# python-microscopy/ch-shrinkwrap

Hardware: NVIDIA B200
Metric: localisation_iterations_per_s (higher is better)
Workload: dtype f32 (fp64 nearest-face compare and Gram sums, int64 fixed-point adjoint)

## Files before the change

ch_shrinkwrap_b200/csrc/common.cuh:

```cuda
#pragma once
#include <cuda_runtime.h>
#include <cfloat>
#include <stdint.h>
#include <string>
#include <unordered_map>
#include <vector>
#include "../../include/nanowrap.h"

#define NW_MAX_LEVELS 12
#define NW_MAX_ITERS 4096
#define NW_S2_PTS 4
#define NW_N_STAGES 11

#ifdef NW_BOUNDS_CHECK
#include <cassert>
#define NW_ASSERT(c) assert(c)
#else
#define NW_ASSERT(c) ((void)0)
#endif

struct Box {
    float4 a;
    float4 b;
    float4 c;
// ... 108 lines not shown
    int64_t P_global = 0;
    float *px = nullptr, *py = nullptr, *pz = nullptr;
    double *px64 = nullptr, *py64 = nullptr, *pz64 = nullptr;
    float *sx = nullptr, *sy = nullptr, *sz = nullptr;
    float *wx = nullptr, *wy = nullptr, *wz = nullptr;
    float sinv_scalar = 1.f;
    int reg_mode = 0;
    int weights_mode = 0;
    float wmean = 1.f;
    int has_mask = 0;
    uint8_t *pmask = nullptr;
    int *perm = nullptr;
    int *slot = nullptr;
    float *w0 = nullptr, *w1 = nullptr, *w2 = nullptr;
    float *rx = nullptr, *ry = nullptr, *rz = nullptr;
    float bbox_pts[6] = {0, 0, 0, 0, 0, 0};
    double wn_max = 1.0;
    bool weights_valid = false;

    int M = 0, F = 0;
    float4 *posq = nullptr, *nrmq = nullptr;
    int *faces = nullptr;
    int *nbrT = nullptr;
    int *valence = nullptr;
    uint8_t *valid = nullptr;
    int *stage_nbr = nullptr, *stage_hev = nullptr;
    int *tb_small = nullptr, *tb_i0 = nullptr, *tb_i1 = nullptr;
    unsigned *tb_u0 = nullptr, *tb_u1 = nullptr, *tb_u2 = nullptr;
    int4 *sfaces = nullptr;
    float4 *cent = nullptr;
    Box *boxes = nullptr;
    int *parent_g = nullptr; int2 *kids = nullptr;
    int *leaf_of_slot = nullptr;
    float *node_f = nullptr;
    TreeLevels tl;
    bool seeds_cold = true;
    float *fx = nullptr, *fy = nullptr, *fz = nullptr;
    bool feet_valid = false;
    unsigned *fkeys = nullptr;
    int *fkey_tab = nullptr;
    float key_lo[3] = {0, 0, 0}, key_inv = 0.f;
    unsigned *fcells = nullptr;
    bool points_mode = false;
    double *cent64 = nullptr;
    Box *tboxes = nullptr;
    char *surf_q = nullptr;
    unsigned *surf_bits = nullptr;
    double *surf_dist = nullptr, *surf_closest = nullptr, *surf_part = nullptr;
    int *surf_face = nullptr;
    int64_t topo_gen = 0;
    int64_t sgn_gen = -1;
    int sgn_defects[5] = {0, 0, 0, 0, 0};
    int *sgn_twin = nullptr;
    int *sgn_voff = nullptr, *sgn_vface = nullptr;
    unsigned long long *sgn_k0 = nullptr, *sgn_k1 = nullptr;
    int *sgn_i0 = nullptr, *sgn_i1 = nullptr;
    int *sgn_cnt = nullptr;
    double *sgn_nv = nullptr;
    double *sgn_vpart = nullptr;
    unsigned *sgn_bbox = nullptr;
    uint8_t *sx_flag = nullptr;
    int *sx_last = nullptr;
    unsigned long long *sx_keys = nullptr, *sx_sorted = nullptr;
    unsigned long long *sx_cnt = nullptr;
    int2 *sx_pairs = nullptr;
    unsigned long long *acc = nullptr;
    float4 *Sq = nullptr;
// ... 145 lines not shown
```

ch_shrinkwrap_b200/csrc/tree.cu:

```cuda
#include <cub/cub.cuh>
#include <cfloat>
#include "common.cuh"
#include <thread>
#include <vector>

namespace {

__device__ __forceinline__ float3 centroid_f32(const float4 a, const float4 b, const float4 c) {
    float3 r;
    r.x = __fdiv_rn(__fadd_rn(__fadd_rn(a.x, b.x), c.x), 3.0f);
    r.y = __fdiv_rn(__fadd_rn(__fadd_rn(a.y, b.y), c.y), 3.0f);
    r.z = __fdiv_rn(__fadd_rn(__fadd_rn(a.z, b.z), c.z), 3.0f);
    return r;
}

__global__ void k_pack_vec3(const float *__restrict__ src, int M, float4 *__restrict__ dst) {
    int i = blockIdx.x * blockDim.x + threadIdx.x;
    if (i < M) dst[i] = make_float4(src[3 * i], src[3 * i + 1], src[3 * i + 2], 0.f);
}

__global__ void k_unpack_vec3(const float4 *__restrict__ src, int M, float *__restrict__ dst) {
    int i = blockIdx.x * blockDim.x + threadIdx.x;
    if (i < M) { float4 v = src[i]; dst[3 * i] = v.x; dst[3 * i + 1] = v.y; dst[3 * i + 2] = v.z; }
}
// ... 39 lines not shown
    return points ? make_float3(a.x, a.y, a.z) : centroid_f32(a, b, c);
}

__global__ void k_face_bbox(const int *__restrict__ faces, const float4 *__restrict__ pos, int F, int *__restrict__ out6, bool points) {
    float lo[3] = {FLT_MAX, FLT_MAX, FLT_MAX}, hi[3] = {-FLT_MAX, -FLT_MAX, -FLT_MAX};
    for (int f = blockIdx.x * blockDim.x + threadIdx.x; f < F; f += gridDim.x * blockDim.x) {
        float3 c = centroid_of(points, pos[faces[3 * f]], pos[faces[3 * f + 1]], pos[faces[3 * f + 2]]);
        float v[3] = {c.x, c.y, c.z};
        for (int a = 0; a < 3; ++a) if (v[a] == v[a]) { lo[a] = fminf(lo[a], v[a]); hi[a] = fmaxf(hi[a], v[a]); }
    }
    for (int a = 0; a < 3; ++a)
        for (int o = 16; o; o >>= 1) {
            lo[a] = fminf(lo[a], __shfl_xor_sync(0xffffffffu, lo[a], o));
            hi[a] = fmaxf(hi[a], __shfl_xor_sync(0xffffffffu, hi[a], o));
        }
    if ((threadIdx.x & 31) == 0)
        for (int a = 0; a < 3; ++a) {
            int l = __float_as_int(lo[a]); l = l >= 0 ? l : l ^ 0x7fffffff;
            int u = __float_as_int(hi[a]); u = u >= 0 ? u : u ^ 0x7fffffff;
            atomicMin(out6 + a, l);
            atomicMax(out6 + 3 + a, u);
        }
}

__device__ __forceinline__ unsigned spread10(unsigned v) {
    v &= 0x3ffu;
    v = (v | v << 16) & 0x30000ffu;
    v = (v | v << 8) & 0x300f00fu;
    v = (v | v << 4) & 0x30c30c3u;
    v = (v | v << 2) & 0x9249249u;
    return v;
}

__global__ void k_face_keys(const int *__restrict__ faces, const float4 *__restrict__ pos, int F, float3 lo, float inv,
                            unsigned *__restrict__ keys, int *__restrict__ idx, unsigned *__restrict__ cells, bool points) {
    int f = blockIdx.x * blockDim.x + threadIdx.x;
    if (f >= F) return;
    float3 c = centroid_of(points, pos[faces[3 * f]], pos[faces[3 * f + 1]], pos[faces[3 * f + 2]]);
    unsigned qx = (unsigned)fminf(fmaxf((c.x - lo.x) * inv, 0.f), 1023.f);
    unsigned qy = (unsigned)fminf(fmaxf((c.y - lo.y) * inv, 0.f), 1023.f);
    unsigned qz = (unsigned)fminf(fmaxf((c.z - lo.z) * inv, 0.f), 1023.f);
    cells[f] = qx | (qy << 10) | (qz << 20);
    hilbert_axes_to_transpose(qx, qy, qz, 10);
    keys[f] = (spread10(qx) << 2) | (spread10(qy) << 1) | spread10(qz);
    idx[f] = f;
}

__global__ void k_sorted_faces(const int *__restrict__ faces, const int *__restrict__ order, int F, int4 *__restrict__ sfaces,
                               const unsigned *__restrict__ cells, unsigned *__restrict__ fcells) {
    int i = blockIdx.x * blockDim.x + threadIdx.x;
    if (i >= F) return;
    int f = order[i];
    sfaces[i] = make_int4(faces[3 * f], faces[3 * f + 1], faces[3 * f + 2], f);
    fcells[i] = cells[f];
}

__device__ __forceinline__ void project3(const float3 n, const float4 c, float &pn, float &p1, float &p2) {
    const float3 t1 = nw_tangent_of(n.x, n.y, n.z);
    const float3 t2 = make_float3(n.y * t1.z - n.z * t1.y, n.z * t1.x - n.x * t1.z, n.x * t1.y - n.y * t1.x);
    pn = fmaf(n.x, c.x, fmaf(n.y, c.y, n.z * c.z));
    p1 = fmaf(t1.x, c.x, fmaf(t1.y, c.y, t1.z * c.z));
    p2 = fmaf(t2.x, c.x, fmaf(t2.y, c.y, t2.z * c.z));
}


__global__ void k_level_histogram(const unsigned *__restrict__ keys, int F, int *__restrict__ hist) {
    const int i = blockIdx.x * blockDim.x + threadIdx.x;
    int lvl = 0;
    if (i < F && i > 0) {
        const unsigned x = keys[i] ^ keys[i - 1];
        if (x) lvl = (29 - (31 - __clz(x))) / 3 + 1;
    }
    for (int k = 1; k <= 10; ++k) {
        const unsigned m = __ballot_sync(0xffffffffu, lvl == k);
        if (m && (threadIdx.x & 31) == 0) atomicAdd(&hist[k], __popc(m));
    }
}

__global__ void k_level_flags(const unsigned *__restrict__ keys, int F, int shift, int *__restrict__ flag) {
    const int i = blockIdx.x * blockDim.x + threadIdx.x;
    if (i >= F) return;
    flag[i] = (i == 0) ? 1 : (shift >= 32 ? 0 : ((keys[i] >> shift) != (keys[i - 1] >> shift)));
}

__device__ __forceinline__ bool ends_node(const unsigned *__restrict__ keys, int F, int lvl, int i) {
    return i == F - 1 || ((keys[i] ^ keys[i + 1]) >> (30 - 3 * lvl)) != 0;
}

__global__ void k_level_tables(const unsigned *__restrict__ keys, int F, int lvl, int off_up, const int *__restrict__ id_up,
                               const int *__restrict__ start_up, int off, const int *__restrict__ id, int *__restrict__ start,
                               int *__restrict__ parent_g, int2 *__restrict__ kids, Box *__restrict__ boxes,
                               int *__restrict__ leaf_of_slot) {
    const int i = blockIdx.x * blockDim.x + threadIdx.x;
    if (i >= F) return;
    if (!id) leaf_of_slot[i] = id_up[i] - 1;
    else if (i == 0 || id[i - 1] != id[i]) start[id[i] - 1] = i;
    if (lvl < 0 || !ends_node(keys, F, lvl, i)) return;
    const int p = off_up + id_up[i] - 1, s0 = start_up[id_up[i] - 1];
    const int c0 = id ? off + id[s0] - 1 : s0, c1 = id ? off + id[i] - 1 : i;
    const unsigned last = (lvl == 0 || ends_node(keys, F, lvl - 1, i)) ? 0x80000000u : 0u;
    kids[p] = make_int2(c0, c1 - c0 + 1);
    boxes[p].d.z = __int_as_float((int)((unsigned)c0 | last));
    if (id) for (int c = c0; c <= c1; ++c) parent_g[c] = (int)((unsigned)p | last);
    if (lvl == 0) parent_g[0] = (int)0x80000000u;
}

__global__ void k_refit_centroids(const int4 *__restrict__ sfaces, const float4 *__restrict__ pos, int F, float4 *__restrict__ cent,
                                  const unsigned *__restrict__ fcells, float3 lo, float inv, SolverState *st, bool points) {
    const int i = blockIdx.x * blockDim.x + threadIdx.x;
    float esc = 0.f;
    if (i < F) {
        const int4 sf = sfaces[i];
        const float3 cc = centroid_of(points, pos[sf.x], pos[sf.y], pos[sf.z]);
        cent[i] = make_float4(cc.x, cc.y, cc.z, __int_as_float(sf.w));
        const unsigned cell = fcells[i];
        const float gx = (cc.x - lo.x) * inv, gy = (cc.y - lo.y) * inv, gz = (cc.z - lo.z) * inv;
        const float cx = (float)(cell & 1023u), cy = (float)((cell >> 10) & 1023u), cz = (float)(cell >> 20);
        esc = fmaxf(fmaxf(fmaxf(cx - gx, cx == 1023.f ? 0.f : gx - (cx + 1.f)), fmaxf(cy - gy, cy == 1023.f ? 0.f : gy - (cy + 1.f))),
                    fmaxf(fmaxf(cz - gz, cz == 1023.f ? 0.f : gz - (cz + 1.f)), 0.f));
        if (!(esc >= 0.f)) esc = __int_as_float(0x7f800000);
    }
    const unsigned m = __reduce_max_sync(0xffffffffu, __float_as_uint(esc));
    if ((threadIdx.x & 31) == 0 && m) atomicMax((unsigned *)&st->cell_escape, m);
}

__global__ void __launch_bounds__(256) k_leaf_normals(const int4 *__restrict__ sfaces, const float4 *__restrict__ pos, int F,
                                                      const int *__restrict__ leaf_of_slot, int leaf0, float *__restrict__ nsum) {
    const int i = blockIdx.x * blockDim.x + threadIdx.x;
    if (i >= F) return;
    const int4 sf = sfaces[i];
    const float4 a = pos[sf.x], b = pos[sf.y], d = pos[sf.z];
    const float ux = b.x - a.x, uy = b.y - a.y, uz = b.z - a.z, vx = d.x - a.x, vy = d.y - a.y, vz = d.z - a.z;
    float3 fn = make_float3(uy * vz - uz * vy, uz * vx - ux * vz, ux * vy - uy * vx);
    if (!(fabsf(fn.x) <= FLT_MAX && fabsf(fn.y) <= FLT_MAX && fabsf(fn.z) <= FLT_MAX)) return;
    float *dst = nsum + 3 * (size_t)(leaf0 + leaf_of_slot[i]);
    atomicAdd(dst, fn.x); atomicAdd(dst + 1, fn.y); atomicAdd(dst + 2, fn.z);
}
__global__ void __launch_bounds__(256) k_up_normals(float *__restrict__ nsum, const int2 *__restrict__ kids, int first, int count) {
    const int j = blockIdx.x * blockDim.x + threadIdx.x;
    if (j >= count) return;
    const int2 k = kids[first + j];
    float sx = 0.f, sy = 0.f, sz = 0.f;
    for (int c = k.x; c < k.x + k.y; ++c) {
        const float *s = nsum + 3 * (size_t)c;
        sx += s[0]; sy += s[1]; sz += s[2];
    }
    float *d = nsum + 3 * (size_t)(first + j);
    d[0] = sx; d[1] = sy; d[2] = sz;
}

__global__ void k_key_table(const unsigned *__restrict__ fkeys, int F, int *__restrict__ tab) {
    const int b = blockIdx.x * blockDim.x + threadIdx.x;
    if (b > 32768) return;
    const unsigned long long key = (unsigned long long)b << 15;
    int lo = 0, hi = F;
    while (lo < hi) {
        const int mid = (lo + hi) >> 1;
        if ((unsigned long long)fkeys[mid] < key) lo = mid + 1; else hi = mid;
    }
    tab[b] = lo;
}

__global__ void k_node_frames(Box *__restrict__ boxes, const float *__restrict__ nsum, int first, int count) {
    const int j = blockIdx.x * blockDim.x + threadIdx.x;
    if (j >= count) return;
    const float *s = nsum + 3 * (size_t)(first + j);
    float3 n = make_float3(s[0], s[1], s[2]);
    const float nn = sqrtf(n.x * n.x + n.y * n.y + n.z * n.z);
    n = (nn > 1e-20f && nn <= FLT_MAX) ? make_float3(n.x / nn, n.y / nn, n.z / nn) : make_float3(0.f, 0.f, 1.f);
    Box *b = &boxes[first + j];
    const float3 t1 = nw_tangent_of(n.x, n.y, n.z);
    b->a = make_float4(n.x, t1.x, n.y, t1.y);
    b->b = make_float4(n.z, t1.z, NW_EMPTY_LO, NW_EMPTY_LO);
    b->c = make_float4(n.y * t1.z - n.z * t1.y, n.z * t1.x - n.x * t1.z, n.x * t1.y - n.y * t1.x, NW_EMPTY_HI);
    b->d.x = NW_EMPTY_HI; b->d.y = NW_EMPTY_HI; b->d.w = NW_EMPTY_LO;
}

__global__ void k_reset_extents(Box *__restrict__ boxes, int first, int count) {
    const int j = blockIdx.x * blockDim.x + threadIdx.x;
    if (j >= count) return;
    Box *b = &boxes[first + j];
    b->b.z = NW_EMPTY_LO; b->b.w = NW_EMPTY_LO; b->d.w = NW_EMPTY_LO; b->d.x = NW_EMPTY_HI; b->d.y = NW_EMPTY_HI; b->c.w = NW_EMPTY_HI;
}

__global__ void __launch_bounds__(256) k_extents(const float4 *__restrict__ cent, int F, const int *__restrict__ leaf_of_slot,
                                                 int leaf0, int leaf_level, const int *__restrict__ parent_g, Box *__restrict__ boxes) {
    const int i = blockIdx.x * blockDim.x + threadIdx.x;
    const bool live = i < F;
    const float4 c = live ? cent[i] : make_float4(0.f, 0.f, 0.f, 0.f);
    const bool finite = live && (c.x == c.x) && (c.y == c.y) && (c.z == c.z);
    int node = live ? leaf0 + leaf_of_slot[i] : 0;
    for (int l = leaf_level; l >= 1; --l) {
        nw_merge_extents(boxes, node, live, finite, [&](const Box *b, float (&lo)[3], float (&hi)[3]) {
            const float4 ba = b->a;
            project3(make_float3(ba.x, ba.z, b->b.x), c, lo[0], lo[1], lo[2]);
            hi[0] = lo[0]; hi[1] = lo[1]; hi[2] = lo[2];
        });
        if (live) node = parent_g[node] & 0x7fffffff;
    }
}
__global__ void k_box_decode(Box *__restrict__ boxes, int first, int count, const SolverState *__restrict__ st) {
    int i = blockIdx.x * blockDim.x + threadIdx.x;
    if (i >= count) return;
    nw_decode_box(&boxes[first + i], st->coord_l1 * 1.9073486328125e-6f);
}

#define NW_NMOM 3

inline float ordered_to_float(int v) {
    v = v >= 0 ? v : v ^ 0x7fffffff;
    float f;
    memcpy(&f, &v, 4);
    return f;
}

}

static int set_topology_impl(nw_ctx *h, const float *pos, const float *nrm, const int32_t *faces, const int32_t *nbr,
                             const int32_t *he_vertex, int n_he, const uint8_t *valid, int M, int F, int he_stride = 4);

extern "C" int nw_set_topology(nw_ctx *h, const float *pos, const float *nrm, const int32_t *faces,
                               const int32_t *nbr, const uint8_t *valid, int M, int F) {
    return set_topology_impl(h, pos, nrm, faces, nbr, nullptr, 0, valid, M, F);
}

extern "C" int nw_set_topology_halfedge(nw_ctx *h, const float *pos, const float *nrm, const int32_t *faces,
                                        const int32_t *nbr_halfedge, const int32_t *he_vertex, int n_halfedges,
                                        const uint8_t *valid, int M, int F) {
    if (h && !(he_vertex && n_halfedges > 0)) { h->err = "nw_set_topology_halfedge: missing half-edge table"; return NW_ERR_ARG; }
    return set_topology_impl(h, pos, nrm, faces, nbr_halfedge, he_vertex, n_halfedges, valid, M, F);
}

extern "C" int nw_set_topology_records(nw_ctx *h, const void *vertex_records, const int32_t *faces, const int32_t *he_vertex,
                                       int he_stride_bytes, int n_halfedges, int M, int F) {
    if (h && !(vertex_records && he_vertex && n_halfedges > 0)) { h->err = "nw_set_topology_records: NULL array"; return NW_ERR_ARG; }
    if (h && !(he_stride_bytes >= 4 && he_stride_bytes % 4 == 0)) { h->err = "nw_set_topology_records: he_stride_bytes must be a multiple of 4"; return NW_ERR_ARG; }
    return set_topology_impl(h, (const float *)vertex_records, nullptr, faces, nullptr, he_vertex, n_halfedges, nullptr, M, F, he_stride_bytes);
}

static int seg_begin(nw_ctx *h) {
// ... 72 lines not shown
        NW_CHECK(nw_alloc(h, &h->stage_nbr, (size_t)NW_NEIGHBORSIZE * M));
        NW_CHECK(nw_upload_replicated(h, h->scratchM, pos, sizeof(float) * 3 * (size_t)M));
        NW_CHECK(seg_begin(h));
        k_pack_vec3<<<nw_grid(M, B), B, 0, s>>>(h->scratchM, M, h->posq);
        h->launches += 1;
        NW_CHECK(seg_end(h));
        NW_CUDA(cudaStreamSynchronize(s));
        NW_CHECK(nw_upload_replicated(h, h->scratchM, nrm, sizeof(float) * 3 * (size_t)M));
        NW_CHECK(seg_begin(h));
        k_pack_vec3<<<nw_grid(M, B), B, 0, s>>>(h->scratchM, M, h->nrmq);
        h->launches += 1;
        NW_CHECK(seg_end(h));
        NW_CHECK(nw_upload_replicated(h, h->stage_nbr, nbr, sizeof(int) * NW_NEIGHBORSIZE * (size_t)M));
        NW_CHECK(seg_begin(h));
        k_transpose_nbr<<<nw_grid(M, B), B, 0, s>>>(h->stage_nbr, he_vertex ? h->stage_hev : nullptr, n_he, M, h->nbrT, h->valence);
        h->launches += 1;
        NW_CHECK(seg_end(h));
        if (valid) NW_CHECK(nw_upload_replicated(h, h->valid, valid, (size_t)M));
        else NW_CUDA(cudaMemsetAsync(h->valid, 1, M, s));
    }
    }
    NW_CUDA(cudaStreamSynchronize(s));
    NW_CHECK(seg_begin(h));
    NW_CUDA(cudaMemsetAsync(h->acc, 0, sizeof(unsigned long long) * 4 * M, s));
    NW_CUDA(cudaMemsetAsync(h->Sq, 0, sizeof(float4) * 3 * M, s));
    if (h->slot && h->P) NW_CUDA(cudaMemsetAsync(h->slot, 0xff, sizeof(int) * h->P, s));
    h->seeds_cold = true;
    h->order_stale = true;
    NW_CHECK(nw_tree_build(h));
    NW_CHECK(seg_end(h));
    return nw_comm_agree(h);
}

static int scan_inclusive(nw_ctx *h, const int *in, int *out, int n) {
    size_t tmp = 0;
    cub::DeviceScan::InclusiveSum(nullptr, tmp, in, out, n, h->stream);
    if (tmp > h->cub_tmp_bytes) { NW_CHECK(nw_alloc(h, (char **)&h->cub_tmp, tmp)); h->cub_tmp_bytes = tmp; }
    NW_CUDA(cub::DeviceScan::InclusiveSum(h->cub_tmp, tmp, in, out, n, h->stream));
    h->launches += 2;
    return NW_OK;
}

static int extents_pass(nw_ctx *h) {
    cudaStream_t s = h->stream;
    const int B = 256;
    const TreeLevels &tl = h->tl;
    const int first = tl.off[1], count = tl.off[tl.n_levels - 1] + tl.count[tl.n_levels - 1] - first;
    k_reset_extents<<<nw_grid(count, B), B, 0, s>>>(h->boxes, first, count);
    NW_LAUNCH_CHECK();
    k_extents<<<nw_grid(h->F, B), B, 0, s>>>(h->cent, h->F, h->leaf_of_slot, tl.off[tl.n_levels - 1], tl.n_levels - 1, h->parent_g,
                                             h->boxes);
    NW_LAUNCH_CHECK();
    k_box_decode<<<nw_grid(count, B), B, 0, s>>>(h->boxes, first, count, h->st);
    NW_LAUNCH_CHECK();
    return NW_OK;
}

static void launch_refit_centroids(nw_ctx *h) {
    cudaMemsetAsync(&h->st->cell_escape, 0, sizeof(float), h->stream);
    k_refit_centroids<<<nw_grid(h->F, 256), 256, 0, h->stream>>>(h->sfaces, h->posq, h->F, h->cent, h->fcells,
                                                                 make_float3(h->key_lo[0], h->key_lo[1], h->key_lo[2]), h->key_inv, h->st,
                                                                 h->points_mode);
}

int nw_tree_refit(nw_ctx *h) {
    launch_refit_centroids(h);
    NW_LAUNCH_CHECK();
    return extents_pass(h);
}

int nw_tree_build(nw_ctx *h) {
    cudaStream_t s = h->stream;
    const int B = 256, F = h->F;
    int *&d_bbox = h->tb_small, *&idx = h->tb_i0, *&order = h->tb_i1;
    unsigned *&keys = h->tb_u0, *&keys2 = h->tb_u1;
    NW_CHECK(nw_alloc(h, &d_bbox, 16));
    int init[6] = {0x7fffffff, 0x7fffffff, 0x7fffffff, (int)0x80000000, (int)0x80000000, (int)0x80000000};
    NW_CUDA(cudaMemcpyAsync(d_bbox, init, sizeof(init), cudaMemcpyHostToDevice, s));
    k_face_bbox<<<std::min(nw_grid(F, B), 148 * 4), B, 0, s>>>(h->faces, h->posq, F, d_bbox, h->points_mode);
    int bb[6];
    NW_CUDA(cudaMemcpyAsync(bb, d_bbox, sizeof(bb), cudaMemcpyDeviceToHost, s));
    NW_CUDA(cudaStreamSynchronize(s));
    float lo[3], hi[3];
    for (int a = 0; a < 3; ++a) { lo[a] = ordered_to_float(bb[a]); hi[a] = ordered_to_float(bb[3 + a]); }
    float ext = fmaxf(fmaxf(hi[0] - lo[0], hi[1] - lo[1]), hi[2] - lo[2]);
    float inv = (ext > 0.f && ext < FLT_MAX) ? 1023.f / ext : 0.f;
    NW_CHECK(nw_alloc(h, &keys, (size_t)F)); NW_CHECK(nw_alloc(h, &keys2, (size_t)F));
    NW_CHECK(nw_alloc(h, &idx, (size_t)F)); NW_CHECK(nw_alloc(h, &order, (size_t)F));
    unsigned *&cells = h->tb_u2;
    NW_CHECK(nw_alloc(h, &cells, (size_t)F)); NW_CHECK(nw_alloc(h, &h->fcells, (size_t)F));
    k_face_keys<<<nw_grid(F, B), B, 0, s>>>(h->faces, h->posq, F, make_float3(lo[0], lo[1], lo[2]), inv, keys, idx, cells, h->points_mode);
    size_t tmp = 0;
    cub::DeviceRadixSort::SortPairs(nullptr, tmp, keys, keys2, idx, order, F, 0, 30, s);
    if (tmp > h->cub_tmp_bytes) { NW_CHECK(nw_alloc(h, (char **)&h->cub_tmp, tmp)); h->cub_tmp_bytes = tmp; }
    NW_CUDA(cub::DeviceRadixSort::SortPairs(h->cub_tmp, tmp, keys, keys2, idx, order, F, 0, 30, s));
    NW_CHECK(nw_alloc(h, &h->fkeys, (size_t)F));
    NW_CUDA(cudaMemcpyAsync(h->fkeys, keys2, sizeof(unsigned) * F, cudaMemcpyDeviceToDevice, s));
    NW_CHECK(nw_alloc(h, &h->fkey_tab, (size_t)32769));
    k_key_table<<<nw_grid(32769, B), B, 0, s>>>(h->fkeys, F, h->fkey_tab);
    h->key_lo[0] = lo[0]; h->key_lo[1] = lo[1]; h->key_lo[2] = lo[2]; h->key_inv = inv;
    k_sorted_faces<<<nw_grid(F, B), B, 0, s>>>(h->faces, order, F, h->sfaces, cells, h->fcells);
    h->launches += 7;

    int *hist = d_bbox;
    NW_CUDA(cudaMemsetAsync(hist, 0, sizeof(int) * 16, s));
    k_level_histogram<<<nw_grid(F, B), B, 0, s>>>(h->fkeys, F, hist);
    int hh[16];
    NW_CUDA(cudaMemcpyAsync(hh, hist, sizeof(hh), cudaMemcpyDeviceToHost, s));
    NW_CUDA(cudaStreamSynchronize(s));
    int cnt[11];
    cnt[0] = 1;
    for (int k = 1; k <= 10; ++k) cnt[k] = cnt[k - 1] + hh[k];
    int kL = 1;
    const double occ = 3.0;
    for (int k = 1; k <= 10; ++k) if ((double)F / cnt[k] >= occ) kL = k;
    TreeLevels &tl = h->tl;
    tl.n_levels = kL + 1;
    int off = 0;
    for (int k = 0; k <= kL; ++k) {
        tl.count[k] = cnt[k]; tl.off[k] = off;
        off += cnt[k];
    }
    const int total = off;
    const size_t room = std::max((size_t)total + total / 4, (size_t)F + F / 2) + 64;
    NW_CHECK(nw_alloc(h, &h->boxes, room)); NW_CHECK(nw_alloc(h, &h->parent_g, room)); NW_CHECK(nw_alloc(h, &h->kids, room));
    NW_CHECK(nw_alloc(h, &h->leaf_of_slot, (size_t)F));
    NW_CHECK(nw_alloc(h, &h->node_f, (size_t)NW_NMOM * room));
    int *flag = idx, *id_cur = order, *id_prev = (int *)keys, *start_cur = (int *)keys2, *start_prev = (int *)cells;
    for (int k = 0; k <= kL; ++k) {
        k_level_flags<<<nw_grid(F, B), B, 0, s>>>(h->fkeys, F, 30 - 3 * k, flag);
        NW_LAUNCH_CHECK();
        NW_CHECK(scan_inclusive(h, flag, id_cur, F));
        k_level_tables<<<nw_grid(F, B), B, 0, s>>>(h->fkeys, F, k - 1, k ? tl.off[k - 1] : 0, id_prev, start_prev, tl.off[k], id_cur,
                                                   start_cur, h->parent_g, h->kids, h->boxes, h->leaf_of_slot);
        NW_LAUNCH_CHECK();
        std::swap(id_cur, id_prev);
        std::swap(start_cur, start_prev);
    }
    k_level_tables<<<nw_grid(F, B), B, 0, s>>>(h->fkeys, F, kL, tl.off[kL], id_prev, start_prev, 0, nullptr, nullptr, h->parent_g,
                                               h->kids, h->boxes, h->leaf_of_slot);
    NW_LAUNCH_CHECK();
    launch_refit_centroids(h);
    NW_LAUNCH_CHECK();
    NW_CUDA(cudaMemsetAsync(h->node_f, 0, sizeof(float) * NW_NMOM * total, s));
    k_leaf_normals<<<nw_grid(F, B), B, 0, s>>>(h->sfaces, h->posq, F, h->leaf_of_slot, tl.off[kL], h->node_f);
    NW_LAUNCH_CHECK();
    for (int k = kL - 1; k >= 0; --k) {
        k_up_normals<<<nw_grid(tl.count[k], B), B, 0, s>>>(h->node_f, h->kids, tl.off[k], tl.count[k]);
        NW_LAUNCH_CHECK();
    }
    k_node_frames<<<nw_grid(total, B), B, 0, s>>>(h->boxes, h->node_f, 0, total);
    NW_LAUNCH_CHECK();
    NW_CHECK(extents_pass(h));
    return NW_OK;
}

namespace {
template <typename T>
__global__ void k_targets_unpack(const T *__restrict__ xyz, int N, float4 *__restrict__ posq, int *__restrict__ faces) {
    const int i = blockIdx.x * blockDim.x + threadIdx.x;
    if (i >= N) return;
    posq[i] = make_float4((float)xyz[3 * (size_t)i], (float)xyz[3 * (size_t)i + 1], (float)xyz[3 * (size_t)i + 2], 0.f);
    faces[3 * (size_t)i] = faces[3 * (size_t)i + 1] = faces[3 * (size_t)i + 2] = i;
}
__global__ void k_targets_sorted64(const double *__restrict__ xyz, const int4 *__restrict__ sfaces, int N, double *__restrict__ cent64) {
    const int s = blockIdx.x * blockDim.x + threadIdx.x;
    if (s >= N) return;
    const size_t i = (size_t)sfaces[s].w;
    cent64[3 * (size_t)s] = xyz[3 * i]; cent64[3 * (size_t)s + 1] = xyz[3 * i + 1]; cent64[3 * (size_t)s + 2] = xyz[3 * i + 2];
}
}

extern "C" int nw_set_point_targets(nw_ctx *h, const void *xyz, int is_f64, int64_t N) {
    if (!h) return NW_ERR_ARG;
    NW_ARG(xyz && N > 0 && N < 2147483647LL / 3, "nw_set_point_targets: need 1 <= N < 2^31 / 3 points");
    NW_ARG(h->nranks == 1, "nw_set_point_targets: single-rank handles only");
    NW_CUDA(cudaSetDevice(h->device));
    cudaStream_t s = h->stream;
    const int n = (int)N, B = 256;
    h->M = n; h->F = n;
    h->epoch++;
    h->topo_gen++;
    h->weights_valid = false; h->pin_fresh = false; h->feet_valid = false;
    h->points_mode = true;
// ... 97 lines not shown
```

Before: 3.365 billion.

## Restructure tree build: fused level scans, single host sync, bottom-up node frames

Tree build now computes Morton-key bounding-box parameters on device so key generation and sorting run without a host round-trip, and replaces the per-level flag/scan/table kernel loop with a block-level multi-level ballot scan plus one prefix kernel. Per-level upward normal sums and the separate node-frame and extents-reset kernels are folded into a bottom-up atomic-counter traversal and into the refit kernel. This cuts launches and one host sync per build, at the cost of more complex kernels that rely on threadfence-ordered atomics.

```diff
diff --git a/ch_shrinkwrap_b200/csrc/common.cuh b/ch_shrinkwrap_b200/csrc/common.cuh
--- a/ch_shrinkwrap_b200/csrc/common.cuh
+++ b/ch_shrinkwrap_b200/csrc/common.cuh
@@ -164,7 +164,7 @@
     Box *boxes = nullptr;
     int *parent_g = nullptr; int2 *kids = nullptr;
     int *leaf_of_slot = nullptr;
-    float *node_f = nullptr;
+    float4 *node_f = nullptr;
     TreeLevels tl;
     bool seeds_cold = true;
     float *fx = nullptr, *fy = nullptr, *fz = nullptr;
diff --git a/ch_shrinkwrap_b200/csrc/tree.cu b/ch_shrinkwrap_b200/csrc/tree.cu
--- a/ch_shrinkwrap_b200/csrc/tree.cu
+++ b/ch_shrinkwrap_b200/csrc/tree.cu
@@ -95,10 +95,19 @@
     return v;
 }
 
-__global__ void k_face_keys(const int *__restrict__ faces, const float4 *__restrict__ pos, int F, float3 lo, float inv,
+__device__ __forceinline__ void key_grid(const int *__restrict__ bb, float3 &lo, float &inv) {
+    lo = make_float3(ord2f(bb[0]), ord2f(bb[1]), ord2f(bb[2]));
+    const float ext = fmaxf(fmaxf(__fsub_rn(ord2f(bb[3]), lo.x), __fsub_rn(ord2f(bb[4]), lo.y)), __fsub_rn(ord2f(bb[5]), lo.z));
+    inv = (ext > 0.f && ext < FLT_MAX) ? __fdiv_rn(1023.f, ext) : 0.f;
+}
+
+__global__ void k_face_keys(const int *__restrict__ faces, const float4 *__restrict__ pos, int F, const int *__restrict__ bb,
                             unsigned *__restrict__ keys, int *__restrict__ idx, unsigned *__restrict__ cells, bool points) {
     int f = blockIdx.x * blockDim.x + threadIdx.x;
     if (f >= F) return;
+    float3 lo;
+    float inv;
+    key_grid(bb, lo, inv);
     float3 c = centroid_of(points, pos[faces[3 * f]], pos[faces[3 * f + 1]], pos[faces[3 * f + 2]]);
     unsigned qx = (unsigned)fminf(fmaxf((c.x - lo.x) * inv, 0.f), 1023.f);
     unsigned qy = (unsigned)fminf(fmaxf((c.y - lo.y) * inv, 0.f), 1023.f);
@@ -118,59 +127,138 @@
     fcells[i] = cells[f];
 }
 
-__device__ __forceinline__ void project3(const float3 n, const float4 c, float &pn, float &p1, float &p2) {
-    const float3 t1 = nw_tangent_of(n.x, n.y, n.z);
-    const float3 t2 = make_float3(n.y * t1.z - n.z * t1.y, n.z * t1.x - n.x * t1.z, n.x * t1.y - n.y * t1.x);
-    pn = fmaf(n.x, c.x, fmaf(n.y, c.y, n.z * c.z));
-    p1 = fmaf(t1.x, c.x, fmaf(t1.y, c.y, t1.z * c.z));
-    p2 = fmaf(t2.x, c.x, fmaf(t2.y, c.y, t2.z * c.z));
-}
-
-
-__global__ void k_level_histogram(const unsigned *__restrict__ keys, int F, int *__restrict__ hist) {
+
+#define NW_KEY_LEVELS 10
+__device__ __forceinline__ int first_diff_level(const unsigned *__restrict__ keys, int i) {
+    if (i == 0) return 0;
+    const unsigned x = keys[i] ^ keys[i - 1];
+    return x ? (29 - (31 - __clz(x))) / 3 + 1 : NW_KEY_LEVELS + 1;
+}
+
+#define NW_LEVEL_B 256
+__device__ __forceinline__ int warp_inclusive_sum(int x) {
+    const int lane = threadIdx.x & 31;
+#pragma unroll
+    for (int o = 1; o < 32; o <<= 1) {
+        const int y = __shfl_up_sync(0xffffffffu, x, o);
+        if (lane >= o) x += y;
+    }
+    return x;
+}
+__device__ __forceinline__ void level_ids(const unsigned *__restrict__ keys, int F, int i, const int *__restrict__ prefix,
+                                          int (&id)[NW_KEY_LEVELS]) {
+    __shared__ int warp_n[NW_LEVEL_B / 32][NW_KEY_LEVELS];
+    const int d = i < F ? first_diff_level(keys, i) : NW_KEY_LEVELS + 1;
+    const int lane = threadIdx.x & 31, w = threadIdx.x >> 5;
+#pragma unroll
+    for (int k = 0; k < NW_KEY_LEVELS; ++k) {
+        const unsigned m = __ballot_sync(0xffffffffu, d <= k + 1);
+        id[k] = __popc(m & (0xffffffffu >> (31 - lane)));
+        if (lane == 0) warp_n[w][k] = __popc(m);
+    }
+    __syncthreads();
+    if (w == 0)
+#pragma unroll
+        for (int k = 0; k < NW_KEY_LEVELS; ++k) {
+            const int v = lane < NW_LEVEL_B / 32 ? warp_n[lane][k] : 0, x = warp_inclusive_sum(v);
+            if (lane < NW_LEVEL_B / 32) warp_n[lane][k] = x - v + (prefix ? prefix[blockIdx.x * NW_KEY_LEVELS + k] : 0);
+        }
+    __syncthreads();
+#pragma unroll
+    for (int k = 0; k < NW_KEY_LEVELS; ++k) id[k] += warp_n[w][k];
+}
+
+__global__ void __launch_bounds__(NW_LEVEL_B) k_level_counts(const unsigned *__restrict__ keys, int F, int *__restrict__ counts) {
+    int id[NW_KEY_LEVELS];
+    level_ids(keys, F, blockIdx.x * NW_LEVEL_B + threadIdx.x, nullptr, id);
+    if (threadIdx.x == NW_LEVEL_B - 1)
+#pragma unroll
+        for (int k = 0; k < NW_KEY_LEVELS; ++k) counts[blockIdx.x * NW_KEY_LEVELS + k] = id[k];
+}
+
+__global__ void __launch_bounds__(1024) k_level_prefix(int *__restrict__ counts, int nblk, int *__restrict__ total) {
+    __shared__ int warp_n[32][NW_KEY_LEVELS], pass_n[NW_KEY_LEVELS];
+    const int lane = threadIdx.x & 31, w = threadIdx.x >> 5;
+    int carry[NW_KEY_LEVELS];
+#pragma unroll
+    for (int k = 0; k < NW_KEY_LEVELS; ++k) carry[k] = 0;
+    for (int r0 = 0; r0 < nblk; r0 += 1024) {
+        const int r = r0 + threadIdx.x;
+        int v[NW_KEY_LEVELS], x[NW_KEY_LEVELS];
+#pragma unroll
+        for (int k = 0; k < NW_KEY_LEVELS; ++k) {
+            v[k] = r < nblk ? counts[r * NW_KEY_LEVELS + k] : 0;
+            x[k] = warp_inclusive_sum(v[k]);
+            if (lane == 31) warp_n[w][k] = x[k];
+        }
+        __syncthreads();
+        if (w == 0)
+#pragma unroll
+            for (int k = 0; k < NW_KEY_LEVELS; ++k) {
+                const int t = warp_n[lane][k], u = warp_inclusive_sum(t);
+                warp_n[lane][k] = u - t;
+                if (lane == 31) pass_n[k] = u;
+            }
+        __syncthreads();
+#pragma unroll
+        for (int k = 0; k < NW_KEY_LEVELS; ++k) {
+            if (r < nblk) counts[r * NW_KEY_LEVELS + k] = carry[k] + warp_n[w][k] + x[k] - v[k];
+            carry[k] += pass_n[k];
+        }
+        __syncthreads();
+    }
+    if (threadIdx.x == 0)
+#pragma unroll
+        for (int k = 0; k < NW_KEY_LEVELS; ++k) total[k] = carry[k];
+}
+
+__device__ __forceinline__ int node_of(const TreeLevels &tl, const int (&id)[NW_KEY_LEVELS], int k) {
+    return tl.off[k] + (k ? id[k - 1] : 1) - 1;
+}
+
+__global__ void __launch_bounds__(NW_LEVEL_B) k_level_first(const unsigned *__restrict__ keys, int F, const __grid_constant__ TreeLevels tl,
+                                                            const int *__restrict__ prefix, int2 *__restrict__ kids) {
+    const int i = blockIdx.x * NW_LEVEL_B + threadIdx.x;
+    int id[NW_KEY_LEVELS];
+    level_ids(keys, F, i, prefix, id);
+    if (i >= F) return;
+    const int kL = tl.n_levels - 1, d = first_diff_level(keys, i);
+#pragma unroll
+    for (int k = 0; k <= NW_KEY_LEVELS; ++k)
+        if (k >= d && k <= kL) kids[node_of(tl, id, k)].x = k < kL ? node_of(tl, id, k < NW_KEY_LEVELS ? k + 1 : k) : i;
+}
+
+__global__ void __launch_bounds__(NW_LEVEL_B) k_level_tables(const unsigned *__restrict__ keys, int F, const __grid_constant__ TreeLevels tl,
+                                                             const int *__restrict__ prefix, int *__restrict__ parent_g,
+                                                             int2 *__restrict__ kids, Box *__restrict__ boxes, int *__restrict__ leaf_of_slot) {
+    const int i = blockIdx.x * NW_LEVEL_B + threadIdx.x;
+    int id[NW_KEY_LEVELS];
+    level_ids(keys, F, i, prefix, id);
+    if (i >= F) return;
+    const int kL = tl.n_levels - 1;
+    const int e = i == F - 1 ? 0 : first_diff_level(keys, i + 1);
+#pragma unroll
+    for (int k = 0; k <= NW_KEY_LEVELS; ++k) {
+        if (k == kL) leaf_of_slot[i] = node_of(tl, id, k) - tl.off[k];
+        if (k < e || k > kL) continue;
+        const int p = node_of(tl, id, k);
+        const int c0 = kids[p].x, c1 = k < kL ? node_of(tl, id, k < NW_KEY_LEVELS ? k + 1 : k) : i;
+        const unsigned last = (k == 0 || k > e) ? 0x80000000u : 0u;
+        kids[p].y = c1 - c0 + 1;
+        boxes[p].d.z = __int_as_float((int)((unsigned)c0 | last));
+        if (k < kL) for (int c = c0; c <= c1; ++c) parent_g[c] = (int)((unsigned)p | last);
+    }
+    if (i == F - 1) parent_g[0] = (int)0x80000000u;
+}
+
+__global__ void k_refit_centroids(const int4 *__restrict__ sfaces, const float4 *__restrict__ pos, int F, float4 *__restrict__ cent,
+                                  const unsigned *__restrict__ fcells, float3 lo, float inv, SolverState *st, bool points,
+                                  Box *__restrict__ boxes, int first, int count) {
     const int i = blockIdx.x * blockDim.x + threadIdx.x;
-    int lvl = 0;
-    if (i < F && i > 0) {
-        const unsigned x = keys[i] ^ keys[i - 1];
-        if (x) lvl = (29 - (31 - __clz(x))) / 3 + 1;
-    }
-    for (int k = 1; k <= 10; ++k) {
-        const unsigned m = __ballot_sync(0xffffffffu, lvl == k);
-        if (m && (threadIdx.x & 31) == 0) atomicAdd(&hist[k], __popc(m));
-    }
-}
-
-__global__ void k_level_flags(const unsigned *__restrict__ keys, int F, int shift, int *__restrict__ flag) {
-    const int i = blockIdx.x * blockDim.x + threadIdx.x;
-    if (i >= F) return;
-    flag[i] = (i == 0) ? 1 : (shift >= 32 ? 0 : ((keys[i] >> shift) != (keys[i - 1] >> shift)));
-}
-
-__device__ __forceinline__ bool ends_node(const unsigned *__restrict__ keys, int F, int lvl, int i) {
-    return i == F - 1 || ((keys[i] ^ keys[i + 1]) >> (30 - 3 * lvl)) != 0;
-}
-
-__global__ void k_level_tables(const unsigned *__restrict__ keys, int F, int lvl, int off_up, const int *__restrict__ id_up,
-                               const int *__restrict__ start_up, int off, const int *__restrict__ id, int *__restrict__ start,
-                               int *__restrict__ parent_g, int2 *__restrict__ kids, Box *__restrict__ boxes,
-                               int *__restrict__ leaf_of_slot) {
-    const int i = blockIdx.x * blockDim.x + threadIdx.x;
-    if (i >= F) return;
-    if (!id) leaf_of_slot[i] = id_up[i] - 1;
-    else if (i == 0 || id[i - 1] != id[i]) start[id[i] - 1] = i;
-    if (lvl < 0 || !ends_node(keys, F, lvl, i)) return;
-    const int p = off_up + id_up[i] - 1, s0 = start_up[id_up[i] - 1];
-    const int c0 = id ? off + id[s0] - 1 : s0, c1 = id ? off + id[i] - 1 : i;
-    const unsigned last = (lvl == 0 || ends_node(keys, F, lvl - 1, i)) ? 0x80000000u : 0u;
-    kids[p] = make_int2(c0, c1 - c0 + 1);
-    boxes[p].d.z = __int_as_float((int)((unsigned)c0 | last));
-    if (id) for (int c = c0; c <= c1; ++c) parent_g[c] = (int)((unsigned)p | last);
-    if (lvl == 0) parent_g[0] = (int)0x80000000u;
-}
-
-__global__ void k_refit_centroids(const int4 *__restrict__ sfaces, const float4 *__restrict__ pos, int F, float4 *__restrict__ cent,
-                                  const unsigned *__restrict__ fcells, float3 lo, float inv, SolverState *st, bool points) {
-    const int i = blockIdx.x * blockDim.x + threadIdx.x;
+    for (int j = i; j < count; j += gridDim.x * blockDim.x) {
+        Box *b = &boxes[first + j];
+        b->b.z = NW_EMPTY_LO; b->b.w = NW_EMPTY_LO; b->d.w = NW_EMPTY_LO; b->d.x = NW_EMPTY_HI; b->d.y = NW_EMPTY_HI; b->c.w = NW_EMPTY_HI;
+    }
     float esc = 0.f;
     if (i < F) {
         const int4 sf = sfaces[i];
@@ -187,30 +275,6 @@
     if ((threadIdx.x & 31) == 0 && m) atomicMax((unsigned *)&st->cell_escape, m);
 }
 
-__global__ void __launch_bounds__(256) k_leaf_normals(const int4 *__restrict__ sfaces, const float4 *__restrict__ pos, int F,
-                                                      const int *__restrict__ leaf_of_slot, int leaf0, float *__restrict__ nsum) {
-    const int i = blockIdx.x * blockDim.x + threadIdx.x;
-    if (i >= F) return;
-    const int4 sf = sfaces[i];
-    const float4 a = pos[sf.x], b = pos[sf.y], d = pos[sf.z];
-    const float ux = b.x - a.x, uy = b.y - a.y, uz = b.z - a.z, vx = d.x - a.x, vy = d.y - a.y, vz = d.z - a.z;
-    float3 fn = make_float3(uy * vz - uz * vy, uz * vx - ux * vz, ux * vy - uy * vx);
-    if (!(fabsf(fn.x) <= FLT_MAX && fabsf(fn.y) <= FLT_MAX && fabsf(fn.z) <= FLT_MAX)) return;
-    float *dst = nsum + 3 * (size_t)(leaf0 + leaf_of_slot[i]);
-    atomicAdd(dst, fn.x); atomicAdd(dst + 1, fn.y); atomicAdd(dst + 2, fn.z);
-}
-__global__ void __launch_bounds__(256) k_up_normals(float *__restrict__ nsum, const int2 *__restrict__ kids, int first, int count) {
-    const int j = blockIdx.x * blockDim.x + threadIdx.x;
-    if (j >= count) return;
-    const int2 k = kids[first + j];
-    float sx = 0.f, sy = 0.f, sz = 0.f;
-    for (int c = k.x; c < k.x + k.y; ++c) {
-        const float *s = nsum + 3 * (size_t)c;
-        sx += s[0]; sy += s[1]; sz += s[2];
-    }
-    float *d = nsum + 3 * (size_t)(first + j);
-    d[0] = sx; d[1] = sy; d[2] = sz;
-}
 
 __global__ void k_key_table(const unsigned *__restrict__ fkeys, int F, int *__restrict__ tab) {
     const int b = blockIdx.x * blockDim.x + threadIdx.x;
@@ -224,14 +288,9 @@
     tab[b] = lo;
 }
 
-__global__ void k_node_frames(Box *__restrict__ boxes, const float *__restrict__ nsum, int first, int count) {
-    const int j = blockIdx.x * blockDim.x + threadIdx.x;
-    if (j >= count) return;
-    const float *s = nsum + 3 * (size_t)(first + j);
-    float3 n = make_float3(s[0], s[1], s[2]);
+__device__ __forceinline__ void node_frame(Box *__restrict__ b, float3 n) {
     const float nn = sqrtf(n.x * n.x + n.y * n.y + n.z * n.z);
     n = (nn > 1e-20f && nn <= FLT_MAX) ? make_float3(n.x / nn, n.y / nn, n.z / nn) : make_float3(0.f, 0.f, 1.f);
-    Box *b = &boxes[first + j];
     const float3 t1 = nw_tangent_of(n.x, n.y, n.z);
     b->a = make_float4(n.x, t1.x, n.y, t1.y);
     b->b = make_float4(n.z, t1.z, NW_EMPTY_LO, NW_EMPTY_LO);
@@ -239,11 +298,41 @@
     b->d.x = NW_EMPTY_HI; b->d.y = NW_EMPTY_HI; b->d.w = NW_EMPTY_LO;
 }
 
-__global__ void k_reset_extents(Box *__restrict__ boxes, int first, int count) {
+__global__ void __launch_bounds__(256) k_leaf_normals(const int4 *__restrict__ sfaces, const float4 *__restrict__ pos, int F,
+                                                      const int *__restrict__ leaf_of_slot, int leaf0, float4 *__restrict__ nsum) {
+    const int i = blockIdx.x * blockDim.x + threadIdx.x;
+    if (i >= F) return;
+    const int4 sf = sfaces[i];
+    const float4 a = pos[sf.x], b = pos[sf.y], d = pos[sf.z];
+    const float ux = b.x - a.x, uy = b.y - a.y, uz = b.z - a.z, vx = d.x - a.x, vy = d.y - a.y, vz = d.z - a.z;
+    float3 fn = make_float3(uy * vz - uz * vy, uz * vx - ux * vz, ux * vy - uy * vx);
+    if (!(fabsf(fn.x) <= FLT_MAX && fabsf(fn.y) <= FLT_MAX && fabsf(fn.z) <= FLT_MAX)) return;
+    float4 *dst = nsum + leaf0 + leaf_of_slot[i];
+    atomicAdd(&dst->x, fn.x); atomicAdd(&dst->y, fn.y); atomicAdd(&dst->z, fn.z);
+}
+__global__ void __launch_bounds__(256) k_node_frames(int leaf0, int n_leaves, const int *__restrict__ parent_g,
+                                                     const int2 *__restrict__ kids, float4 *nsum, Box *__restrict__ boxes) {
     const int j = blockIdx.x * blockDim.x + threadIdx.x;
-    if (j >= count) return;
-    Box *b = &boxes[first + j];
-    b->b.z = NW_EMPTY_LO; b->b.w = NW_EMPTY_LO; b->d.w = NW_EMPTY_LO; b->d.x = NW_EMPTY_HI; b->d.y = NW_EMPTY_HI; b->c.w = NW_EMPTY_HI;
+    if (j >= n_leaves) return;
+    int node = leaf0 + j;
+    const float4 l = nsum[node];
+    float3 s = make_float3(l.x, l.y, l.z);
+    for (;;) {
+        node_frame(&boxes[node], s);
+        if (node == 0) return;
+        const int p = parent_g[node] & 0x7fffffff;
+        __threadfence();
+        if (atomicAdd((int *)&nsum[p].w, 1) != kids[p].y - 1) return;
+        __threadfence();
+        const int2 k = kids[p];
+        s = make_float3(0.f, 0.f, 0.f);
+        for (int c = k.x; c < k.x + k.y; ++c) {
+            const float4 v = __ldcg(&nsum[c]);
+            s.x += v.x; s.y += v.y; s.z += v.z;
+        }
+        __stcg(&nsum[p].x, s.x); __stcg(&nsum[p].y, s.y); __stcg(&nsum[p].z, s.z);
+        node = p;
+    }
 }
 
 __global__ void __launch_bounds__(256) k_extents(const float4 *__restrict__ cent, int F, const int *__restrict__ leaf_of_slot,
@@ -255,8 +344,11 @@
     int node = live ? leaf0 + leaf_of_slot[i] : 0;
     for (int l = leaf_level; l >= 1; --l) {
         nw_merge_extents(boxes, node, live, finite, [&](const Box *b, float (&lo)[3], float (&hi)[3]) {
-            const float4 ba = b->a;
-            project3(make_float3(ba.x, ba.z, b->b.x), c, lo[0], lo[1], lo[2]);
+            const float4 ba = b->a, bc = b->c;
+            const float2 bb = make_float2(b->b.x, b->b.y);
+            lo[0] = fmaf(ba.x, c.x, fmaf(ba.z, c.y, bb.x * c.z));
+            lo[1] = fmaf(ba.y, c.x, fmaf(ba.w, c.y, bb.y * c.z));
+            lo[2] = fmaf(bc.x, c.x, fmaf(bc.y, c.y, bc.z * c.z));
             hi[0] = lo[0]; hi[1] = lo[1]; hi[2] = lo[2];
         });
         if (live) node = parent_g[node] & 0x7fffffff;
@@ -267,8 +359,6 @@
     if (i >= count) return;
     nw_decode_box(&boxes[first + i], st->coord_l1 * 1.9073486328125e-6f);
 }
-
-#define NW_NMOM 3
 
 inline float ordered_to_float(int v) {
     v = v >= 0 ? v : v ^ 0x7fffffff;
@@ -407,22 +497,11 @@
     return nw_comm_agree(h);
 }
 
-static int scan_inclusive(nw_ctx *h, const int *in, int *out, int n) {
-    size_t tmp = 0;
-    cub::DeviceScan::InclusiveSum(nullptr, tmp, in, out, n, h->stream);
-    if (tmp > h->cub_tmp_bytes) { NW_CHECK(nw_alloc(h, (char **)&h->cub_tmp, tmp)); h->cub_tmp_bytes = tmp; }
-    NW_CUDA(cub::DeviceScan::InclusiveSum(h->cub_tmp, tmp, in, out, n, h->stream));
-    h->launches += 2;
-    return NW_OK;
-}
-
 static int extents_pass(nw_ctx *h) {
     cudaStream_t s = h->stream;
     const int B = 256;
     const TreeLevels &tl = h->tl;
     const int first = tl.off[1], count = tl.off[tl.n_levels - 1] + tl.count[tl.n_levels - 1] - first;
-    k_reset_extents<<<nw_grid(count, B), B, 0, s>>>(h->boxes, first, count);
-    NW_LAUNCH_CHECK();
     k_extents<<<nw_grid(h->F, B), B, 0, s>>>(h->cent, h->F, h->leaf_of_slot, tl.off[tl.n_levels - 1], tl.n_levels - 1, h->parent_g,
                                              h->boxes);
     NW_LAUNCH_CHECK();
@@ -432,10 +511,12 @@
 }
 
 static void launch_refit_centroids(nw_ctx *h) {
+    const TreeLevels &tl = h->tl;
+    const int first = tl.off[1], count = tl.off[tl.n_levels - 1] + tl.count[tl.n_levels - 1] - first;
     cudaMemsetAsync(&h->st->cell_escape, 0, sizeof(float), h->stream);
     k_refit_centroids<<<nw_grid(h->F, 256), 256, 0, h->stream>>>(h->sfaces, h->posq, h->F, h->cent, h->fcells,
                                                                  make_float3(h->key_lo[0], h->key_lo[1], h->key_lo[2]), h->key_inv, h->st,
-                                                                 h->points_mode);
+                                                                 h->points_mode, h->boxes, first, count);
 }
 
 int nw_tree_refit(nw_ctx *h) {
@@ -447,48 +528,50 @@
 int nw_tree_build(nw_ctx *h) {
     cudaStream_t s = h->stream;
     const int B = 256, F = h->F;
-    int *&d_bbox = h->tb_small, *&idx = h->tb_i0, *&order = h->tb_i1;
-    unsigned *&keys = h->tb_u0, *&keys2 = h->tb_u1;
-    NW_CHECK(nw_alloc(h, &d_bbox, 16));
-    int init[6] = {0x7fffffff, 0x7fffffff, 0x7fffffff, (int)0x80000000, (int)0x80000000, (int)0x80000000};
+    int *&idx = h->tb_i0, *&order = h->tb_i1;
+    unsigned *&keys = h->tb_u0, *&keys2 = h->tb_u1, *&cells = h->tb_u2;
+    NW_CHECK(nw_alloc(h, &keys, (size_t)F)); NW_CHECK(nw_alloc(h, &keys2, (size_t)F));
+    const int nblk = nw_grid(F, NW_LEVEL_B);
+    NW_CHECK(nw_alloc(h, &idx, (size_t)std::max(F, nblk * NW_KEY_LEVELS))); NW_CHECK(nw_alloc(h, &order, (size_t)F));
+    NW_CHECK(nw_alloc(h, &cells, (size_t)F)); NW_CHECK(nw_alloc(h, &h->fcells, (size_t)F));
+    NW_CHECK(nw_alloc(h, &h->fkeys, (size_t)F));
+    NW_CHECK(nw_alloc(h, &h->fkey_tab, (size_t)32769));
+    int *&small = h->tb_small;
+    NW_CHECK(nw_alloc(h, &small, 32));
+    int *d_bbox = small;
+    const int init[6] = {0x7fffffff, 0x7fffffff, 0x7fffffff, (int)0x80000000, (int)0x80000000, (int)0x80000000};
     NW_CUDA(cudaMemcpyAsync(d_bbox, init, sizeof(init), cudaMemcpyHostToDevice, s));
     k_face_bbox<<<std::min(nw_grid(F, B), 148 * 4), B, 0, s>>>(h->faces, h->posq, F, d_bbox, h->points_mode);
-    int bb[6];
-    NW_CUDA(cudaMemcpyAsync(bb, d_bbox, sizeof(bb), cudaMemcpyDeviceToHost, s));
+    k_face_keys<<<nw_grid(F, B), B, 0, s>>>(h->faces, h->posq, F, d_bbox, keys, idx, cells, h->points_mode);
+    size_t tmp = 0;
+    cub::DeviceRadixSort::SortPairs(nullptr, tmp, keys, keys2, idx, order, F, 0, 30, s);
+    if (tmp > h->cub_tmp_bytes) { NW_CHECK(nw_alloc(h, (char **)&h->cub_tmp, tmp)); h->cub_tmp_bytes = tmp; }
+    NW_CUDA(cub::DeviceRadixSort::SortPairs(h->cub_tmp, tmp, keys, keys2, idx, order, F, 0, 30, s));
+    NW_CUDA(cudaMemcpyAsync(h->fkeys, keys2, sizeof(unsigned) * F, cudaMemcpyDeviceToDevice, s));
+    k_key_table<<<nw_grid(32769, B), B, 0, s>>>(h->fkeys, F, h->fkey_tab);
+    k_sorted_faces<<<nw_grid(F, B), B, 0, s>>>(h->faces, order, F, h->sfaces, cells, h->fcells);
+    h->launches += 7;
+    int *prefix = idx;
+    k_level_counts<<<nblk, NW_LEVEL_B, 0, s>>>(h->fkeys, F, prefix);
+    NW_LAUNCH_CHECK();
+    k_level_prefix<<<1, 1024, 0, s>>>(prefix, nblk, small + 8);
+    NW_LAUNCH_CHECK();
+    int back[18];
+    NW_CUDA(cudaMemcpyAsync(back, small, sizeof(back), cudaMemcpyDeviceToHost, s));
     NW_CUDA(cudaStreamSynchronize(s));
+
+    const int *bb = back;
     float lo[3], hi[3];
     for (int a = 0; a < 3; ++a) { lo[a] = ordered_to_float(bb[a]); hi[a] = ordered_to_float(bb[3 + a]); }
     float ext = fmaxf(fmaxf(hi[0] - lo[0], hi[1] - lo[1]), hi[2] - lo[2]);
     float inv = (ext > 0.f && ext < FLT_MAX) ? 1023.f / ext : 0.f;
-    NW_CHECK(nw_alloc(h, &keys, (size_t)F)); NW_CHECK(nw_alloc(h, &keys2, (size_t)F));
-    NW_CHECK(nw_alloc(h, &idx, (size_t)F)); NW_CHECK(nw_alloc(h, &order, (size_t)F));
-    unsigned *&cells = h->tb_u2;
-    NW_CHECK(nw_alloc(h, &cells, (size_t)F)); NW_CHECK(nw_alloc(h, &h->fcells, (size_t)F));
-    k_face_keys<<<nw_grid(F, B), B, 0, s>>>(h->faces, h->posq, F, make_float3(lo[0], lo[1], lo[2]), inv, keys, idx, cells, h->points_mode);
-    size_t tmp = 0;
-    cub::DeviceRadixSort::SortPairs(nullptr, tmp, keys, keys2, idx, order, F, 0, 30, s);
-    if (tmp > h->cub_tmp_bytes) { NW_CHECK(nw_alloc(h, (char **)&h->cub_tmp, tmp)); h->cub_tmp_bytes = tmp; }
-    NW_CUDA(cub::DeviceRadixSort::SortPairs(h->cub_tmp, tmp, keys, keys2, idx, order, F, 0, 30, s));
-    NW_CHECK(nw_alloc(h, &h->fkeys, (size_t)F));
-    NW_CUDA(cudaMemcpyAsync(h->fkeys, keys2, sizeof(unsigned) * F, cudaMemcpyDeviceToDevice, s));
-    NW_CHECK(nw_alloc(h, &h->fkey_tab, (size_t)32769));
-    k_key_table<<<nw_grid(32769, B), B, 0, s>>>(h->fkeys, F, h->fkey_tab);
     h->key_lo[0] = lo[0]; h->key_lo[1] = lo[1]; h->key_lo[2] = lo[2]; h->key_inv = inv;
-    k_sorted_faces<<<nw_grid(F, B), B, 0, s>>>(h->faces, order, F, h->sfaces, cells, h->fcells);
-    h->launches += 7;
-
-    int *hist = d_bbox;
-    NW_CUDA(cudaMemsetAsync(hist, 0, sizeof(int) * 16, s));
-    k_level_histogram<<<nw_grid(F, B), B, 0, s>>>(h->fkeys, F, hist);
-    int hh[16];
-    NW_CUDA(cudaMemcpyAsync(hh, hist, sizeof(hh), cudaMemcpyDeviceToHost, s));
-    NW_CUDA(cudaStreamSynchronize(s));
-    int cnt[11];
+    int cnt[NW_KEY_LEVELS + 1];
     cnt[0] = 1;
-    for (int k = 1; k <= 10; ++k) cnt[k] = cnt[k - 1] + hh[k];
+    for (int k = 1; k <= NW_KEY_LEVELS; ++k) cnt[k] = back[8 + k - 1];
     int kL = 1;
     const double occ = 3.0;
-    for (int k = 1; k <= 10; ++k) if ((double)F / cnt[k] >= occ) kL = k;
+    for (int k = 1; k <= NW_KEY_LEVELS; ++k) if ((double)F / cnt[k] >= occ) kL = k;
     TreeLevels &tl = h->tl;
     tl.n_levels = kL + 1;
     int off = 0;
@@ -500,31 +583,17 @@
     const size_t room = std::max((size_t)total + total / 4, (size_t)F + F / 2) + 64;
     NW_CHECK(nw_alloc(h, &h->boxes, room)); NW_CHECK(nw_alloc(h, &h->parent_g, room)); NW_CHECK(nw_alloc(h, &h->kids, room));
     NW_CHECK(nw_alloc(h, &h->leaf_of_slot, (size_t)F));
-    NW_CHECK(nw_alloc(h, &h->node_f, (size_t)NW_NMOM * room));
-    int *flag = idx, *id_cur = order, *id_prev = (int *)keys, *start_cur = (int *)keys2, *start_prev = (int *)cells;
-    for (int k = 0; k <= kL; ++k) {
-        k_level_flags<<<nw_grid(F, B), B, 0, s>>>(h->fkeys, F, 30 - 3 * k, flag);
-        NW_LAUNCH_CHECK();
-        NW_CHECK(scan_inclusive(h, flag, id_cur, F));
-        k_level_tables<<<nw_grid(F, B), B, 0, s>>>(h->fkeys, F, k - 1, k ? tl.off[k - 1] : 0, id_prev, start_prev, tl.off[k], id_cur,
-                                                   start_cur, h->parent_g, h->kids, h->boxes, h->leaf_of_slot);
-        NW_LAUNCH_CHECK();
-        std::swap(id_cur, id_prev);
-        std::swap(start_cur, start_prev);
-    }
-    k_level_tables<<<nw_grid(F, B), B, 0, s>>>(h->fkeys, F, kL, tl.off[kL], id_prev, start_prev, 0, nullptr, nullptr, h->parent_g,
-                                               h->kids, h->boxes, h->leaf_of_slot);
+    NW_CHECK(nw_alloc(h, &h->node_f, room));
+    k_level_first<<<nblk, NW_LEVEL_B, 0, s>>>(h->fkeys, F, tl, prefix, h->kids);
+    NW_LAUNCH_CHECK();
+    k_level_tables<<<nblk, NW_LEVEL_B, 0, s>>>(h->fkeys, F, tl, prefix, h->parent_g, h->kids, h->boxes, h->leaf_of_slot);
     NW_LAUNCH_CHECK();
     launch_refit_centroids(h);
     NW_LAUNCH_CHECK();
-    NW_CUDA(cudaMemsetAsync(h->node_f, 0, sizeof(float) * NW_NMOM * total, s));
+    NW_CUDA(cudaMemsetAsync(h->node_f, 0, sizeof(float4) * total, s));
     k_leaf_normals<<<nw_grid(F, B), B, 0, s>>>(h->sfaces, h->posq, F, h->leaf_of_slot, tl.off[kL], h->node_f);
     NW_LAUNCH_CHECK();
-    for (int k = kL - 1; k >= 0; --k) {
-        k_up_normals<<<nw_grid(tl.count[k], B), B, 0, s>>>(h->node_f, h->kids, tl.off[k], tl.count[k]);
-        NW_LAUNCH_CHECK();
-    }
-    k_node_frames<<<nw_grid(total, B), B, 0, s>>>(h->boxes, h->node_f, 0, total);
+    k_node_frames<<<nw_grid(tl.count[kL], B), B, 0, s>>>(tl.off[kL], tl.count[kL], h->parent_g, h->kids, h->node_f, h->boxes);
     NW_LAUNCH_CHECK();
     NW_CHECK(extents_pass(h));
     return NW_OK;
```

Measured after the change: 3.429 billion (median of 6 runs). 1.02x the previous value.
